# ka9q/ka9q-radio

Hardware: NVIDIA H100
Metric: input Msamples/s through forward+filter+inverse at N channels (higher is better)
Workload: dtype f32

## Files before the change

### ka9q_radio_b200/csrc/static_kernels_v2.cuh

```cuda
#pragma once
#include "static_kernels.cuh"

namespace kfft {

__device__ __forceinline__ void unpack_i16(int raw, int &lo, int &hi) {
  asm("prmt.b32 %0, %1, 0, 0x9910;" : "=r"(lo) : "r"(raw));
  hi = raw >> 16;
}
__device__ __forceinline__ float i32_to_f32(int v) {
  float f;
  asm("cvt.rn.f32.s32 %0, %1;" : "=f"(f) : "r"(v));
  return f;
}

template <bool REAL_SPLIT>
struct RowsV2Shape {
  using P = SPlan<1250, 10, 25, 5>;
  static constexpr int N2 = 1250, PITCH = 1250, GT = 256, SKEW = 2;
  static constexpr int NG = REAL_SPLIT ? 2 : 1, T = GT * NG, COLS = 8 * NG;
  static constexpr int IPC = REAL_SPLIT ? COLS / 2 : COLS;
  static constexpr int TW = (static_tw_count<P>() + 1) & ~1;
  static constexpr int TILE = COLS * PITCH + (NG - 1) * SKEW;
  static constexpr size_t smem = sizeof(float2) * (size_t)(TILE + TW);
  static __host__ __device__ constexpr int col_off(int c) { return c * PITCH + (c >> 3) * SKEW; }
};

__device__ constexpr float kRowsTw0[3][4][2] = {
    {{9.870916009e-01f, -1.601568460e-01f}, {9.486995935e-01f, -3.161789477e-01f}, {8.000617623e-01f, -5.999176502e-01f}, {2.801976204e-01f, -9.599423409e-01f}},
    {{9.486995935e-01f, -3.161789477e-01f}, {8.000617623e-01f, -5.999176502e-01f}, {2.801976204e-01f, -9.599423409e-01f}, {-8.429785967e-01f, -5.379471183e-01f}},
    {{8.858151436e-01f, -4.640382826e-01f}, {5.693368912e-01f, -8.221042752e-01f}, {-3.517109454e-01f, -9.361086488e-01f}, {-7.525988221e-01f, 6.584793329e-01f}},
};

template <bool REAL_SPLIT, int N1C = 0, bool HALVED = false>
__global__ void __launch_bounds__(RowsV2Shape<REAL_SPLIT>::T, REAL_SPLIT ? 1 : 2) fwd_rows_v2(Pass2Args const a, FwdTables const tb) {
  using S = RowsV2Shape<REAL_SPLIT>;
  using P = typename S::P;
  constexpr int N2 = S::N2, T = S::T, GT = S::GT, COLS = S::COLS, IPC = S::IPC;
  constexpr int R0 = 10, S0 = 125, R1 = 25, NSUB1 = 125, S1 = 5, R2 = 5;
  extern __shared__ __align__(16) unsigned char smem_raw[];
  float2 *tile = reinterpret_cast<float2 *>(smem_raw);
  float2 *s_tw = tile + S::TILE;
  __shared__ __align__(8) uint64_t bars[COLS];
  __shared__ __align__(8) uint64_t tbar;
  TilePlan const &pl = c_plans[a.plan];
  int const tid = threadIdx.x, lane = tid & 31, warp = tid >> 5;
  int const blk = gridDim.y - 1 - blockIdx.y;
  int const n1 = N1C ? N1C : a.n1;
  int const item0 = blockIdx.x * IPC;
  auto row_of = [&](int col) -> int {
    RowItem const it = row_item(item0 + (REAL_SPLIT ? col >> 1 : col), n1, REAL_SPLIT);
    if (REAL_SPLIT) {
      if ((col & 1) == 0) return it.kind != kRowEmpty ? it.row_a : -1;
      return it.kind == kRowPair ? it.row_b : -1;
    }
    return it.kind == kRowPlain ? it.row_a : -1;
  };
  if (lane == 0) {
    int const row = row_of(warp);
    mbar_init(&bars[warp], 1);
    if (warp == 0) mbar_init(&tbar, 1);
    mbar_fence_init();
    if (row >= 0) {
      mbar_expect_tx(&bars[warp], N2 * 8);
      bulk_g2s(tile + S::col_off(warp), a.mid + ((long)blk * n1 + row) * a.mid_ld, N2 * 8, &bars[warp]);
    }
    if (warp == 0) {
      constexpr uint32_t TWB = (uint32_t)S::TW * 8u;
      mbar_expect_tx(&tbar, TWB);
      bulk_g2s(s_tw, pl.tw, TWB, &tbar);
    }
  }
  __syncthreads();
  int const g = tid / GT;
  int const c = (tid & 7) + 8 * g, ul = (tid % GT) >> 3;
  auto group_sync = [&] {
    if (S::NG == 1) __syncthreads();
    else asm volatile("bar.sync %0, %1;" ::"r"(1 + g), "n"(GT) : "memory");
  };
  bool const col_ok = row_of(c) >= 0;
  mbar_wait(&tbar, 0);
  if (col_ok) mbar_wait(&bars[c], 0);
  float2 *mycol = tile + S::col_off(c);

  if (col_ok) {
    float2 base[4];
#pragma unroll
    for (int q = 0; q < 4; q++) base[q] = s_tw[((1 << q) - 1) * S0 + ul];
#pragma unroll
    for (int it = 0; it < 4; it++) {
      int const j = ul + (GT / 8) * it;
      if (it < 3 || j < S0) {
        float2 *p = mycol + j;
        float2 x[R0], w[R0];
#pragma unroll
        for (int m = 0; m < R0; m++) x[m] = p[m * S0];
#pragma unroll
        for (int q = 0; q < 4; q++)
          w[1 << q] = it == 0 ? base[q] : cmul(base[q], make_float2(kRowsTw0[it > 0 ? it - 1 : 0][q][0], kRowsTw0[it > 0 ? it - 1 : 0][q][1]));
        w[3] = cmul(w[2], w[1]);
        w[5] = cmul(w[4], w[1]);
        w[6] = cmul(w[4], w[2]);
        w[7] = cmul(w[4], w[3]);
        w[9] = cmul(w[8], w[1]);
        Dft<R0, false>::run(x);
        p[0] = x[0];
#pragma unroll
        for (int t = 1; t < R0; t++) p[t * S0] = cmul(x[t], w[t]);
      }
    }
  }
  group_sync();
  if (col_ok) {
    float2 const *tw1 = s_tw + P::tw_off(1);
#pragma unroll 1
    for (int u = ul; u < N2 / R1; u += GT / 8) {
      int const b = u / S1, j = u - b * S1;
      float2 *p = mycol + b * NSUB1 + j;
      float2 x[R1];
#pragma unroll
      for (int m = 0; m < R1; m++) x[m] = p[m * S1];
      Dft<R1, false>::run(x);
#pragma unroll
      for (int t = 1; t < R1; t++) x[t] = cmul(x[t], tw1[(t - 1) * S1 + j]);
#pragma unroll
      for (int t = 0; t < R1; t++) p[t * S1] = x[t];
    }
  }
  constexpr int UQ = T / IPC;
  int const i = tid % IPC, uq = tid / IPC;
  RowItem const it = row_item(item0 + i, n1, REAL_SPLIT);
  float2 rootC = make_float2(1.f, 0.f), rd[4];
  bool self_item = false;
  if (REAL_SPLIT) {
    self_item = it.kind == kRowSelf0 || it.kind == kRowSelfMid;
    if (it.kind == kRowPair) rootC = __ldg(tb.rootC + it.row_a);
#pragma unroll
    for (int q = 0; q < 4; q++) {
      int const u = uq + UQ * q;
      int const t0 = u / 25, t1 = u - t0 * 25;
      rd[q] = (it.kind == kRowPair && u < N2 / R2) ? __ldg(a.rootD + t0 + 10 * t1) : make_float2(1.f, 0.f);
    }
  }
  int const has_self = __syncthreads_or(self_item);

  float2 *spec = a.spec + (long)blk * a.spec_stride;
  float const hf = HALVED ? 1.0f : 0.5f;
  if (!REAL_SPLIT) {
    if (col_ok) {
      float2 *dst = spec + row_of(c);
#pragma unroll 1
      for (int u = ul; u < N2 / R2; u += GT / 8) {
        int const t0 = u / 25, t1 = u - t0 * 25;
        int const kb = t0 + 10 * t1;
        float2 const *p = mycol + u * R2;
        float2 x[R2];
#pragma unroll
        for (int m = 0; m < R2; m++) x[m] = p[m];
        Dft<R2, false>::run(x);
        float2 *d = dst + (long)n1 * kb;
#pragma unroll
        for (int t = 0; t < R2; t++) d[(long)n1 * 250 * t] = x[t];
      }
    }
    return;
  }
  int const nc = N1C ? N1C * N2 : (int)a.nc;
  if (it.kind == kRowPair) {
    float2 const *ca = tile + S::col_off(2 * i), *cb = tile + S::col_off(2 * i + 1);
#pragma unroll
    for (int q = 0; q < 4; q++) {
      int const u = uq + UQ * q;
      if (u >= N2 / R2) break;
      int const t0 = u / 25, t1 = u - t0 * 25;
      int const kb = t0 + 10 * t1;
      float2 const wkb = cmul(rootC, rd[q]);
      float2 za[R2], zb[R2];
      float2 const *pa = ca + u * R2, *pb = cb + (N2 / R2 - 1 - u) * R2;
      float2 *pk = spec + (it.row_a + n1 * kb), *pm = spec + (nc - it.row_a - n1 * kb);
#pragma unroll
      for (int m = 0; m < R2; m++) {
        za[m] = pa[m];
        zb[m] = pb[m];
      }
      Dft<R2, false>::run(za);
      Dft<R2, false>::run(zb);
#pragma unroll
      for (int t = 0; t < R2; t++) {
        float2 const A = za[t], B = zb[R2 - 1 - t];
        float2 const w = (t == 0) ? wkb : cmul(wkb, wroot<10>(t));
        float2 const E = HALVED ? make_float2(A.x + B.x, A.y - B.y) : make_float2(0.5f * (A.x + B.x), 0.5f * (A.y - B.y));
        float2 const O = HALVED ? make_float2(A.x - B.x, A.y + B.y) : make_float2(0.5f * (A.x - B.x), 0.5f * (A.y + B.y));
        float2 const Pp = cmul(w, O);
        pk[(long)n1 * 250 * t] = make_float2(E.x + Pp.y, E.y - Pp.x);
        pm[-(long)n1 * 250 * t] = make_float2(E.x - Pp.y, -(E.y + Pp.x));
      }
    }
  }
  if (!has_self) return;
  for (int s = 0; s < IPC; s++) {
    RowItem const its = row_item(item0 + s, n1, true);
    if (its.kind != kRowSelf0 && its.kind != kRowSelfMid) continue;
    float2 *col = tile + S::col_off(2 * s);
    for (int u = tid; u < N2 / R2; u += T) {
      float2 x[R2];
#pragma unroll
      for (int m = 0; m < R2; m++) x[m] = col[u * R2 + m];
      Dft<R2, false>::run(x);
#pragma unroll
      for (int m = 0; m < R2; m++) col[u * R2 + m] = x[m];
    }
  }
  __syncthreads();
  for (int s = 0; s < IPC; s++) {
    RowItem const its = row_item(item0 + s, n1, true);
    if (its.kind != kRowSelf0 && its.kind != kRowSelfMid) continue;
    float2 const *col = tile + S::col_off(2 * s);
    float2 const rC = __ldg(tb.rootC + its.row_a);
    bool const self0 = its.kind == kRowSelf0;
    int const kend = self0 ? N2 / 2 + 1 : (N2 + 1) / 2;
    for (int k2 = tid; k2 < kend; k2 += T) {
      int const k2m = self0 ? (k2 == 0 ? 0 : N2 - k2) : N2 - 1 - k2;
      float2 const A = col[static_slot<P>(k2)], B = col[static_slot<P>(k2m)];
      float2 const w = cmul(rC, __ldg(a.rootD + k2));
      float2 const E = make_float2(hf * (A.x + B.x), hf * (A.y - B.y));
      float2 const O = make_float2(hf * (A.x - B.x), hf * (A.y + B.y));
      float2 const Pp = cmul(w, O);
      int const k = its.row_a + n1 * k2;
      spec[k] = make_float2(E.x + Pp.y, E.y - Pp.x);
      if (nc - k != k) spec[nc - k] = make_float2(E.x - Pp.y, -(E.y + Pp.x));
    }
  }
}

template <class P, bool OSC = false>
__global__ void __launch_bounds__(kChanWarps * 32) chan_v2(ChanArgs const a) {
  static_assert(P::nst == 2, "two-stage plans only");
  extern __shared__ __align__(16) unsigned char smem_raw[];
  __shared__ __align__(8) uint64_t bars[kChanWarps];
  __shared__ __align__(8) uint64_t tbar;
  constexpr int NS = P::len, TOP = (NS + 1) / 2, R0 = P::rad(0), R1 = P::rad(1), S0 = NS / R0;
  static_assert(S0 == R1 && NS % 2 == 0, "plan shape");
  constexpr int XS = NS + 4;
  int const lane = threadIdx.x & 31, warp = threadIdx.x >> 5;
  int const oi = blockIdx.x * kChanWarps + warp;
  float2 *s_tw = reinterpret_cast<float2 *>(smem_raw) + kChanWarps * (NS + XS);
  bool const active = oi < a.norder;
  ChanDesc d;
  d.plan = -1;
  if (active) d = a.desc[a.order ? a.order[oi] : a.chan_base + oi];
  if (threadIdx.x == 0) {
    int p0 = -1;
    for (int w = 0; w < kChanWarps && p0 < 0; w++) {
      int const o = blockIdx.x * kChanWarps + w;
      if (o < a.norder) p0 = a.desc[a.order ? a.order[o] : a.chan_base + o].plan;
    }
    mbar_init(&tbar, 1);
    mbar_fence_init();
    if (p0 >= 0) {
      constexpr uint32_t TWB = (uint32_t)((static_tw_count<P>() + 1) & ~1) * 8u;
      mbar_expect_tx(&tbar, TWB);
      bulk_g2s(s_tw, c_plans[p0].tw, TWB, &tbar);
    }
  }
  __syncthreads();
  if (!active || d.plan < 0) return;
  int const blk = blockIdx.y;
  float2 *col = reinterpret_cast<float2 *>(smem_raw) + warp * (NS + XS);
  float2 *xs = col + NS;
  float2 const *X = a.spec + (long)blk * a.spec_stride;
  float2 const *R = a.resp + d.resp_off;
  float2 *dst = a.out + (long)blk * a.out_stride + d.out_off;
  if (d.ncopy <= 0) {
    for (int i = lane; i < d.olen; i += 32) dst[i] = make_float2(0.f, 0.f);
    if ((d.flags & kChanOsc) && a.power && lane == 0) a.power[(long)blk * a.power_stride + (a.order ? a.order[oi] : a.chan_base + oi)] = 0.f;
    mbar_wait(&tbar, 0);
    return;
  }
  int const qlo = d.dir > 0 ? d.q0 : d.q0 - (d.ncopy - 1);
  bool const wraps = a.wrap && (d.q0 + d.ncopy > a.m_bins);
  int const qa = qlo & ~1;
  if (!wraps) {
    int const qhi = qlo + d.ncopy - 1;
    uint32_t const nx = (uint32_t)(((qhi - qa + 1) + 1) & ~1);
    if (lane == 0) {
      mbar_init(&bars[warp], 1);
      mbar_fence_init();
      mbar_expect_tx(&bars[warp], nx * 8 + NS * 8);
      bulk_g2s(xs, X + qa, nx * 8, &bars[warp]);
      bulk_g2s(col, R, NS * 8, &bars[warp]);
    }
    __syncwarp();
    mbar_wait(&bars[warp], 0);
  } else {
    for (int i = lane; i < NS; i += 32) col[i] = __ldg(R + i);
    for (int u = lane; u < d.ncopy; u += 32) {
      int q = d.q0 + u;
      if (q >= a.m_bins) q -= a.m_bins;
      xs[u] = __ldg(X + q);
    }
    __syncwarp();
  }
  mbar_wait(&tbar, 0);
  auto product = [&](int wp) -> float2 {
    int t = wp - TOP;
    if (t < 0) t += NS;
    int const u = t - d.zlead;
    bool const live = (u >= 0 && u < d.ncopy && wp != TOP);
    int const xi = wraps ? u : (d.q0 + d.dir * u - qa);
    float2 x = xs[live ? xi : 0];
    if (d.dir < 0) x.y = -x.y;
    float2 const v = cmul(x, col[wp]);
    return live ? v : make_float2(0.f, 0.f);
  };
  if (d.flags & kChanIsb) {
    for (int wp = lane; wp < NS; wp += 32) col[wp] = product(wp);
    __syncwarp();
    for (int p = 1 + lane; p < NS / 2; p += 32) {
      float2 const pos = col[p], neg = col[NS - p];
      col[p] = make_float2(pos.x + neg.x, pos.y - neg.y);
      col[NS - p] = make_float2(neg.x - pos.x, neg.y + pos.y);
    }
    if (lane == 0) {
      col[0] = make_float2(0.f, 0.f);
      col[TOP] = make_float2(0.f, 0.f);
    }
    __syncwarp();
    static_stage<P, true, 0, true, 1>(col, s_tw, lane);
    __syncwarp();
  } else if (lane < S0) {
    float2 x[R0];
#pragma unroll
    for (int m = 0; m < R0; m++) x[m] = product(lane + S0 * m);
    Dft<R0, true>::run(x);
    col[lane] = x[0];
#pragma unroll
    for (int t = 1; t < R0; t++) col[lane + S0 * t] = cmulc(x[t], s_tw[(t - 1) * S0 + lane]);
  }
  __syncwarp();
  bool const osc = OSC && (d.flags & kChanOsc) != 0;
  float pw = 0.f;
  int const ci = a.order ? a.order[oi] : a.chan_base + oi;
  if (lane < R0) {
    float2 x[R1];
#pragma unroll
    for (int m = 0; m < R1; m++) x[m] = col[R1 * lane + m];
    Dft<R1, true>::run(x);
    int const first = NS - d.olen;
    if (!OSC || !osc) {
#pragma unroll
      for (int t = 0; t < R1; t++) {
        int const n = lane + R0 * t;
        if (n >= first) dst[n - first] = x[t];
      }
    } else if (OSC) {
      ChanAux const ax = a.aux[ci];
      long const k = a.block0 + blk - ax.osc_epoch;
#pragma unroll
      for (int t = 0; t < R1; t++) {
        int const n = lane + R0 * t;
        if (n >= first) {
          float2 const v = osc_rotate(x[t], osc_phase_cycles(ax, k, d.olen, n - first));
          dst[n - first] = v;
          pw += v.x * v.x + v.y * v.y;
        }
      }
    }
  }
  if (OSC && osc && a.power) {
    pw = warp_sum(pw);
    if (lane == 0) a.power[(long)blk * a.power_stride + ci] = pw / (float)d.olen;
  }
}

}
```

Baseline: 91050.

## Add extra pair column group so real-split rows write coalesced mirror outputs

In the real-split row kernel, each block now loads two extra columns (the next item's pair), handled by an extra 64-thread group. The split/mirror output is remapped so each warp covers 8 items plus one extra item. Direct writes go only to items below IPC and mirror writes only to items above zero, so adjacent blocks share the boundary item's mirror outputs and store more contiguously. The cost is more shared memory, more threads, and extra row-FFT work on the duplicated columns.

```diff
diff --git a/ka9q_radio_b200/csrc/static_kernels_v2.cuh b/ka9q_radio_b200/csrc/static_kernels_v2.cuh
--- a/ka9q_radio_b200/csrc/static_kernels_v2.cuh
+++ b/ka9q_radio_b200/csrc/static_kernels_v2.cuh
@@ -16,13 +16,14 @@
 template <bool REAL_SPLIT>
 struct RowsV2Shape {
   using P = SPlan<1250, 10, 25, 5>;
-  static constexpr int N2 = 1250, PITCH = 1250, GT = 256, SKEW = 2;
-  static constexpr int NG = REAL_SPLIT ? 2 : 1, T = GT * NG, COLS = 8 * NG;
-  static constexpr int IPC = REAL_SPLIT ? COLS / 2 : COLS;
+  static constexpr int N2 = 1250, PITCH = 1250, GT = 256, SKEW = 2, XSKEW = 6;
+  static constexpr int NG = REAL_SPLIT ? 2 : 1, XT = REAL_SPLIT ? 64 : 0, T = GT * NG + XT;
+  static constexpr int IPC = 8;
+  static constexpr int COLS = REAL_SPLIT ? 2 * IPC + 2 : IPC;
   static constexpr int TW = (static_tw_count<P>() + 1) & ~1;
-  static constexpr int TILE = COLS * PITCH + (NG - 1) * SKEW;
+  static constexpr int TILE = COLS * PITCH + (REAL_SPLIT ? 2 * SKEW + XSKEW : 0);
   static constexpr size_t smem = sizeof(float2) * (size_t)(TILE + TW);
-  static __host__ __device__ constexpr int col_off(int c) { return c * PITCH + (c >> 3) * SKEW; }
+  static __host__ __device__ constexpr int col_off(int c) { return c * PITCH + (c >> 3) * SKEW + (REAL_SPLIT && c > 16 ? XSKEW : 0); }
 };
 
 __device__ constexpr float kRowsTw0[3][4][2] = {
@@ -50,7 +51,7 @@
   auto row_of = [&](int col) -> int {
     RowItem const it = row_item(item0 + (REAL_SPLIT ? col >> 1 : col), n1, REAL_SPLIT);
     if (REAL_SPLIT) {
-      if ((col & 1) == 0) return it.kind != kRowEmpty ? it.row_a : -1;
+      if ((col & 1) == 0) return (it.kind == kRowPair || (col < 2 * IPC && it.kind != kRowEmpty)) ? it.row_a : -1;
       return it.kind == kRowPair ? it.row_b : -1;
     }
     return it.kind == kRowPlain ? it.row_a : -1;
@@ -72,10 +73,12 @@
   }
   __syncthreads();
   int const g = tid / GT;
-  int const c = (tid & 7) + 8 * g, ul = (tid % GT) >> 3;
+  bool const xg = REAL_SPLIT && g == S::NG;
+  int const c = xg ? 2 * IPC + (tid & 1) : (tid & 7) + 8 * g;
+  int const ul = xg ? (tid - S::NG * GT) >> 1 : (tid % GT) >> 3;
   auto group_sync = [&] {
     if (S::NG == 1) __syncthreads();
-    else asm volatile("bar.sync %0, %1;" ::"r"(1 + g), "n"(GT) : "memory");
+    else asm volatile("bar.sync %0, %1;" ::"r"(1 + g), "r"(xg ? S::XT : GT) : "memory");
   };
   bool const col_ok = row_of(c) >= 0;
   mbar_wait(&tbar, 0);
@@ -126,17 +129,19 @@
       for (int t = 0; t < R1; t++) p[t * S1] = x[t];
     }
   }
-  constexpr int UQ = T / IPC;
-  int const i = tid % IPC, uq = tid / IPC;
-  RowItem const it = row_item(item0 + i, n1, REAL_SPLIT);
-  float2 rootC = make_float2(1.f, 0.f), rd[4];
+  constexpr int US = 3 * (T / 32), NQ = (N2 / R2 + US - 1) / US;
+  int const i = REAL_SPLIT ? (lane < 24 ? lane & 7 : IPC) : tid % IPC;
+  int const uq = REAL_SPLIT ? 3 * warp + (lane < 24 ? lane >> 3 : lane - 24) : 0;
+  RowItem it = row_item(item0 + i, n1, REAL_SPLIT);
+  if (REAL_SPLIT && lane >= 27) it.kind = kRowEmpty;
+  float2 rootC = make_float2(1.f, 0.f), rd[NQ];
   bool self_item = false;
   if (REAL_SPLIT) {
-    self_item = it.kind == kRowSelf0 || it.kind == kRowSelfMid;
+    self_item = i < IPC && (it.kind == kRowSelf0 || it.kind == kRowSelfMid);
     if (it.kind == kRowPair) rootC = __ldg(tb.rootC + it.row_a);
 #pragma unroll
-    for (int q = 0; q < 4; q++) {
-      int const u = uq + UQ * q;
+    for (int q = 0; q < NQ; q++) {
+      int const u = uq + US * q;
       int const t0 = u / 25, t1 = u - t0 * 25;
       rd[q] = (it.kind == kRowPair && u < N2 / R2) ? __ldg(a.rootD + t0 + 10 * t1) : make_float2(1.f, 0.f);
     }
@@ -167,9 +172,10 @@
   int const nc = N1C ? N1C * N2 : (int)a.nc;
   if (it.kind == kRowPair) {
     float2 const *ca = tile + S::col_off(2 * i), *cb = tile + S::col_off(2 * i + 1);
-#pragma unroll
-    for (int q = 0; q < 4; q++) {
-      int const u = uq + UQ * q;
+    bool const direct = i < IPC, mirror = i > 0;
+#pragma unroll
+    for (int q = 0; q < NQ; q++) {
+      int const u = uq + US * q;
       if (u >= N2 / R2) break;
       int const t0 = u / 25, t1 = u - t0 * 25;
       int const kb = t0 + 10 * t1;
@@ -191,8 +197,8 @@
         float2 const E = HALVED ? make_float2(A.x + B.x, A.y - B.y) : make_float2(0.5f * (A.x + B.x), 0.5f * (A.y - B.y));
         float2 const O = HALVED ? make_float2(A.x - B.x, A.y + B.y) : make_float2(0.5f * (A.x - B.x), 0.5f * (A.y + B.y));
         float2 const Pp = cmul(w, O);
-        pk[(long)n1 * 250 * t] = make_float2(E.x + Pp.y, E.y - Pp.x);
-        pm[-(long)n1 * 250 * t] = make_float2(E.x - Pp.y, -(E.y + Pp.x));
+        if (direct) pk[(long)n1 * 250 * t] = make_float2(E.x + Pp.y, E.y - Pp.x);
+        if (mirror) pm[-(long)n1 * 250 * t] = make_float2(E.x - Pp.y, -(E.y + Pp.x));
       }
     }
   }
```

After: 89230, median of 6. -2.0%, worse.
